# zz9tf/FIA-KDD-19

Hardware: AMD Instinct MI355X
Metric: influence queries/sec (whole node) + % HBM roofline, MF k=16 ML-1M-ex (higher is better)
Workload: dtype f64

## Files before the change

fia-kdd-19_amd/csrc/abi.hip:

```cpp
#include <atomic>
#include <cstdlib>
#include <cstring>
#include <new>

#include "common.h"

namespace fia {

static bool pooled_event(fia_ctx* c, hipEvent_t* e) {
  if (!c->events.pool.empty()) {
    *e = c->events.pool.back();
    c->events.pool.pop_back();
    return true;
  }
  return hipEventCreate(e) == hipSuccess;
}

void phase_begin(fia_ctx* c, int phase, hipStream_t s) {
  if (!(c->profiling >> phase & 1u)) return;
  hipEvent_t a, b;
  if (!pooled_event(c, &a)) return;
  if (!pooled_event(c, &b)) { c->events.pool.push_back(a); return; }
  (void)hipEventRecord(a, s);
  c->events.ev[phase].push_back({a, b});
// ... 178 lines not shown
      if (can_free) b.release(ds);
      else { b.ptr = nullptr; b.bytes = 0; }
    };
    for (int s = 0; s < 2; ++s) {
      for (fia::DevBuf* b : {&c->idx.side[s].ptr, &c->idx.side[s].row, &c->idx.side[s].other, &c->idx.side[s].rating,
                             &c->gram[s], &c->l1[s], &c->idx.order[s], &c->idx.gitems[s], &c->idx.gcomb[s],
                             &c->gpart[s], &c->self[s], &c->gm[s], &c->slot[s], &c->bitems[s], &c->bcomb[s]})
        rel(*b);
    }
    fia::DevBuf* bufs[] = {&c->rec,    &c->coff,   &c->cdesc,    &c->cand_pos,  &c->cand_val, &c->qscan,
                           &c->flag,   &c->nch,    &c->coupled,  &c->idx.pkey,  &c->idx.pcnt, &c->idx.psum,
                           &c->gcnt,   &c->gstart, &c->grank,    &c->gq,        &c->qbase,    &c->gscan,
                           &c->wstart, &c->witems, &c->resid,  &c->qwork,  &c->xb,       &c->syslist,
                           &c->cpllist, &c->lscr, &c->mark, &c->d1tab, &c->slices, &c->wfrag,
                           &c->tkeys, &c->tvals, &c->tagg, &c->tslot, &c->tword, &c->tsort, &c->rowrec, &c->gxq,
                           &c->dwork, &c->dslab, &c->dpairs};
    for (auto* b : bufs) rel(*b);
    if (can_free) (void)hipStreamSynchronize(ds);
    if (c->aux && !capturing) (void)hipStreamDestroy(c->aux);
    if (c->fork_ev) (void)hipEventDestroy(c->fork_ev);
    if (c->l1_ev) (void)hipEventDestroy(c->l1_ev);
    if (c->prep_ev) (void)hipEventDestroy(c->prep_ev);
    for (auto& v : c->events.ev)
      for (auto& pr : v) { (void)hipEventDestroy(pr.first); (void)hipEventDestroy(pr.second); }
    for (auto e : c->events.pool) (void)hipEventDestroy(e);
  }
  if (c->device >= 0 && c->device < kMaxDevices) g_live[c->device].fetch_sub(1);
  delete c;
  return FIA_OK;
}

// ... 628 lines not shown
```

fia-kdd-19_amd/csrc/common.h:

```cpp
#pragma once

#include <hip/hip_runtime.h>
#include <hip/hip_ext.h>
#include <cstdint>
#include <cstdio>
#include <string>
#include <vector>

#include "fia.h"

namespace fia {

constexpr int kWave = 64;
constexpr int kScoreThreads = 256;
constexpr int kScoreRows = 4;
constexpr int kChunk = 64 * kScoreRows;
constexpr int kRunQB = 16;
constexpr int kRunChunk = 128;
constexpr int kNcfRunChunk = 64;
constexpr int kRunUserCost = 3;

struct ChunkDesc {
  int64_t list_base;
  int64_t out_base;
// ... 182 lines not shown
  fia::Params p;
  fia::Index idx;
  fia::DevBuf gram[2];
  fia::DevBuf l1[2];
  fia::DevBuf gpart[2];
  bool prepared = false;
  fia::DevBuf rec;
  fia::DevBuf coff;
  fia::DevBuf cdesc;
  fia::DevBuf cand_pos;
  fia::DevBuf cand_val;
  fia::DevBuf qscan;
  fia::DevBuf flag;
  fia::DevBuf nch;
  fia::DevBuf coupled;
  fia::DevBuf gcnt;
  fia::DevBuf gstart;
  fia::DevBuf grank;
  fia::DevBuf gq;
  fia::DevBuf qbase;
  fia::DevBuf slices;
  fia::DevBuf wstart;
  fia::DevBuf gscan;
  fia::DevBuf witems;
  fia::DevBuf d1tab;
  fia::DevBuf tkeys, tvals, tagg, tslot, tword, tsort;
  fia::DevBuf rowrec, gxq;
  uint64_t rowrec_version = ~0ull;
  fia::DevBuf dwork, dslab, dpairs;
  fia::DevBuf self[2];
// ... 114 lines not shown
  const int2* desc;
  const uint32_t* ids;
  const int32_t* wave;
  int64_t n_waves;
  const float* emb_other[2];
  uint32_t bytes_other[2];
  double* gram[2];
  double* part[2];
  const uint8_t* mark;
  int64_t moff[2];
};
hipError_t launch_gram_mf_stream(int k, const GramStreamArgs& G, hipStream_t s);
hipError_t launch_score_mf_runs(int k, int64_t grid, hipStream_t s, const QueryArgs& A, int64_t Q,
                                const ChunkDesc* cdesc, const int64_t* qbase, const int32_t* slices,
                                const double* rec, int32_t* rel_idx, double* influence, int K, int32_t* cand_pos,
                                double* cand_val, PhaseSpan ps);
hipError_t launch_score_ncf_runs(int k, int64_t grid, hipStream_t s, const QueryArgs& A, int64_t Q,
                                 const ChunkDesc* cdesc, const int64_t* qbase, const int32_t* slices,
                                 const double* rec, int32_t* rel_idx, double* influence, int K, int32_t* cand_pos,
                                 double* cand_val, PhaseSpan ps);
hipError_t launch_score_mf_mfma(int k, bool full, int64_t grid, hipStream_t s, PhaseSpan ps, const QueryArgs& A,
                                int64_t nE, const int64_t* wstart, const int32_t* witems, const int64_t* gstart,
                                const int32_t* gq, const int64_t* qbase, const double* rec, int32_t* rel_idx,
                                double* influence, int K, int32_t* cand_pos, double* cand_val);
hipError_t launch_topk_merge(fia_ctx* c, int64_t Q, const int32_t* qu, const int32_t* qi, int K, int spc,
                             int64_t* topk_pos, int64_t* topk_idx, double* topk_val, hipStream_t s,
                             int64_t max_chunks);

hipError_t score_candidates(fia_ctx* c, int64_t Q, const int32_t* qu, const int32_t* qi, const double* x,
                            const int64_t* cand_offsets, int64_t total_cand, const int32_t* cand_user,
                            const int32_t* cand_item, const float* cand_rating, double* influence, int K,
// ... 74 lines not shown
```

fia-kdd-19_amd/csrc/index.hip:

```cpp
#include <algorithm>
#include <cstdlib>
#include <cstring>
#include <rocprim/device/device_radix_sort.hpp>
#include <rocprim/iterator/counting_iterator.hpp>

#include "common.h"
#include "scan.h"

namespace fia {
namespace {

__global__ void k_check_ids(const int32_t* __restrict__ user, const int32_t* __restrict__ item, int64_t N,
                            int64_t U, int64_t I, int32_t* __restrict__ flag) {
  int64_t j = (int64_t)blockIdx.x * blockDim.x + threadIdx.x;
  int64_t stride = (int64_t)gridDim.x * blockDim.x;
  int bad = 0;
  for (; j < N; j += stride) {
    int32_t u = user[j], i = item[j];
    bad |= (u < 0 || u >= U || i < 0 || i >= I);
  }
  if (__any(bad) && (threadIdx.x & 63) == 0) atomicOr(flag, 1);
}

__global__ void k_gather_side(const int32_t* __restrict__ rows, const int32_t* __restrict__ other_src,
// ... 46 lines not shown
  ub = du = ib = di = 0;
  if (u >= 0 && u < U && i >= 0 && i < I) {
    ub = uptr[u];
    du = uptr[u + 1] - ub;
    ib = iptr[i];
    di = iptr[i + 1] - ib;
  }
}

template <int MODE>
__global__ __launch_bounds__(kScanThreads) void k_query_scan(
    const int32_t* __restrict__ qu, const int32_t* __restrict__ qi, int64_t Q, const int64_t* __restrict__ uptr,
    const int64_t* __restrict__ iptr, int64_t U, int64_t I, int64_t* __restrict__ out,
    unsigned long long* __restrict__ tstate, unsigned int* __restrict__ tctr, int32_t* __restrict__ flag,
    const int64_t* __restrict__ offsets, ChunkDesc* __restrict__ cdesc, int32_t* __restrict__ zero_word,
    int64_t* __restrict__ qbase, int runs, int clen, int lsh, int32_t* __restrict__ slices) {
  query_scan_body<MODE>(qu, qi, Q, uptr, iptr, U, I, out, tstate, tctr, flag, offsets, cdesc, zero_word, qbase, runs,
                        clen, lsh, slices);
}

__global__ void k_group_count(const int32_t* __restrict__ qu, const int32_t* __restrict__ qi, int64_t Q,
                              const int64_t* __restrict__ uptr, const int64_t* __restrict__ iptr, int64_t U, int64_t I,
                              const int64_t* __restrict__ offsets, const int64_t* __restrict__ coff,
                              unsigned long long* __restrict__ gcnt, int32_t* __restrict__ grank,
                              int64_t* __restrict__ qbase) {
  const int64_t q = (int64_t)blockIdx.x * blockDim.x + threadIdx.x;
  if (q >= Q) return;
  int64_t ub, du, ib, di;
  query_sides(qu, qi, q, uptr, iptr, U, I, ub, du, ib, di);
  const int32_t u = qu[q], i = qi[q];
  const bool ok = (u >= 0 && u < U && i >= 0 && i < I) && (du + di > 0);
  grank[2 * q] = ok ? (int32_t)atomicAdd(&gcnt[u], 1ull) : -1;
  grank[2 * q + 1] = ok ? (int32_t)atomicAdd(&gcnt[U + i], 1ull) : -1;
// ... 398 lines not shown
  X.valid = true;
  return hipSuccess;
}

static hipError_t scan_state(fia_ctx* c, int64_t Q, hipStream_t s) {
  const int64_t ntiles = (Q + 1 + kScanTile - 1) / kScanTile;
  const size_t need = sizeof(unsigned long long) * (size_t)(2 * ntiles) + 16;
  if (c->qscan.bytes >= need && c->qscan.ptr) return hipSuccess;
  FIA_HIP_TRY(c->qscan.reserve(need < 4096 ? 4096 : need, s));
  FIA_HIP_TRY(hipMemsetAsync(c->qscan.ptr, 0, c->qscan.bytes, s));
  return hipSuccess;
}

static hipError_t query_scan_args(fia_ctx* c, int64_t Q, const int32_t* qu, const int32_t* qi, int64_t* out,
                                  const int64_t* offsets, ChunkDesc* cdesc, int32_t* zero_word, hipStream_t s,
                                  int64_t* qbase, int runs, int clen, int lsh, int32_t* slices, ScanArgs& S) {
  FIA_HIP_TRY(scan_state(c, Q, s));
  FIA_HIP_TRY(c->flag.reserve(64, s));
  unsigned int* ctr = reinterpret_cast<unsigned int*>(c->qscan.as<char>() + c->qscan.bytes - 16);
  S = ScanArgs{qu, qi, Q, c->idx.side[0].ptr.as<int64_t>(), c->idx.side[1].ptr.as<int64_t>(), c->idx.U, c->idx.I, out,
               c->qscan.as<unsigned long long>(), ctr, c->flag.as<int32_t>(), offsets, cdesc, zero_word, qbase, runs,
               clen, lsh, slices};
  return hipSuccess;
}

template <int MODE>
static hipError_t launch_query_scan(const ScanArgs& S, hipStream_t s, hipEvent_t ev_a, hipEvent_t ev_b) {
  hipExtLaunchKernelGGL(k_query_scan<MODE>, dim3((unsigned)scan_tiles(S.Q)), dim3(kScanThreads), 0, s, ev_a, ev_b, 0,
                        S.qu, S.qi, S.Q, S.uptr, S.iptr, S.U, S.I, S.out, S.tstate, S.tctr, S.flag, S.offsets, S.cdesc,
                        S.zero_word, S.qbase, S.runs, S.clen, S.lsh, S.slices);
  return hipGetLastError();
}

hipError_t count_related(fia_ctx* c, int64_t Q, const int32_t* qu, const int32_t* qi, int64_t* offsets,
                         hipStream_t s) {
  ScanArgs S;
  FIA_HIP_TRY(query_scan_args(c, Q, qu, qi, offsets, nullptr, nullptr, nullptr, s, nullptr, 0, kChunk, 0, nullptr, S));
  return launch_query_scan<0>(S, s, nullptr, nullptr);
}

hipError_t write_related(fia_ctx* c, int64_t Q, const int32_t* qu, const int32_t* qi, const int64_t* offsets,
                         int32_t* rel, hipStream_t s) {
  if (Q == 0) return hipSuccess;
  hipLaunchKernelGGL(k_write_related, dim3((unsigned)Q), dim3(256), 0, s, qu, qi, offsets,
                     c->idx.side[0].ptr.as<int64_t>(), c->idx.side[0].row.as<int32_t>(),
                     c->idx.side[1].ptr.as<int64_t>(), c->idx.side[1].row.as<int32_t>(), c->idx.U, c->idx.I, rel);
  return hipGetLastError();
}


hipError_t chunk_scan_args(fia_ctx* c, int64_t Q, const int32_t* qu, const int32_t* qi, const int64_t* offsets,
                           int64_t max_chunks, bool offsets_only, hipStream_t s, int32_t* zero_word, bool runs,
                           int slice_cost, int run_chunk, ScanArgs& S) {
  FIA_HIP_TRY(c->coff.reserve(sizeof(int64_t) * (size_t)(Q + 1), s));
  const bool rq = runs && !offsets_only;
  if (!offsets_only) FIA_HIP_TRY(c->cdesc.reserve(sizeof(ChunkDesc) * (size_t)(max_chunks + 1), s));
  int lsh = 0;
  while ((1 << lsh) < slice_cost && lsh < 30) ++lsh;
  const int lam = 1 << lsh;
  if (rq) {
    FIA_HIP_TRY(c->qbase.reserve(sizeof(int64_t) * (size_t)(4 * Q + 2), s));
    FIA_HIP_TRY(c->slices.reserve(sizeof(int32_t) * (size_t)((max_chunks + 1) * (kRunQB + 2) / lam + 2), s));
  }
  return query_scan_args(c, Q, qu, qi, c->coff.as<int64_t>(), offsets,
                         offsets_only ? nullptr : c->cdesc.as<ChunkDesc>(), zero_word, s,
                         rq ? c->qbase.as<int64_t>() : nullptr, rq ? kRunQB : 0, rq ? run_chunk : kChunk, lsh,
                         rq ? c->slices.as<int32_t>() : nullptr, S);
}

hipError_t launch_chunk_scan(const ScanArgs& S, hipStream_t s, hipEvent_t ev_a, hipEvent_t ev_b) {
  return launch_query_scan<1>(S, s, ev_a, ev_b);
}

hipError_t build_chunks(fia_ctx* c, int64_t Q, const int32_t* qu, const int32_t* qi, const int64_t* offsets,
                        int64_t max_chunks, bool offsets_only, hipStream_t s, int32_t* zero_word, bool runs,
                        int slice_cost, int run_chunk) {
  ScanArgs S;
  FIA_HIP_TRY(chunk_scan_args(c, Q, qu, qi, offsets, max_chunks, offsets_only, s, zero_word, runs, slice_cost,
                              run_chunk, S));
  return launch_chunk_scan(S, s);
}

// ... 44 lines not shown
```

fia-kdd-19_amd/csrc/models.hip:

```cpp
#include "kern.h"
#include "scan.h"

namespace fia {

QueryArgs make_args(fia_ctx* c, const int32_t* qu, const int32_t* qi) {
  QueryArgs A{};
  fill_list_args(c, A);
  A.qu = qu;
  A.qi = qi;
  A.lgm[0] = c->gm[0].as<double>();
  A.lgm[1] = c->gm[1].as<double>();
  A.lres = c->resid.as<double>();
  A.N = c->idx.N;
  return A;
}

namespace {

template <class M>
constexpr int kModel = M::ncf ? FIA_MODEL_NCF : FIA_MODEL_MF;

constexpr int kRunLambda = 8;

template <class M>
// ... 76 lines not shown
    FIA_HIP_TRY(c->cand_val.reserve(sizeof(double) * (size_t)((max_chunks + 1) * K * spc), s));
  }
  QueryArgs A = make_args(c, qu, qi);
  const int64_t nE = c->idx.U + c->idx.I;
  const int64_t max_items = max_chunks;
  if (c->coupled.bytes < sizeof(int32_t) * (size_t)(Q + 2) || !c->coupled.ptr) {
    FIA_HIP_TRY(c->coupled.reserve(sizeof(int32_t) * (size_t)(Q + 2), s));
    FIA_HIP_TRY(hipMemsetAsync(c->coupled.ptr, 0, c->coupled.bytes, s));
  }
  int32_t* const coupled = c->coupled.as<int32_t>() + 1;
  constexpr bool ext_phases = runs && !M::ncf && use_quad_solve<M>();
  const bool fused = ext_phases && Q > 0 && !x_in;
  if (!ext_phases) phase_begin(c, 4, s);
  constexpr int64_t lam = kRunLambda;
  const int64_t runs_grid = (kRunUserCost * (max_chunks + 1)) / lam + 2;
  ScanArgs S;
  FIA_HIP_TRY(chunk_scan_args(c, Q, qu, qi, offsets, max_chunks, grouped, s, fused ? nullptr : coupled, runs, (int)lam,
                              M::ncf ? kNcfRunChunk : kRunChunk, S));
  if (!fused) {
    const PhaseSpan cspan = ext_phases ? phase_span(c, 4) : PhaseSpan{};
    if (const hipError_t eb = launch_chunk_scan(S, s, cspan.a, cspan.b); eb != hipSuccess) {
      phase_drop(c, 4, cspan);
      return eb;
    }
  }
  if (grouped) FIA_HIP_TRY(build_groups(c, Q, qu, qi, offsets, max_items, qblock, s, use_mfma ? kMfmaCPI : 1));
  if constexpr (pair_layout<M>()) {
    if (Q > 0 && !x_in) {
      FIA_HIP_TRY(join_l1(c, s));
      FIA_HIP_TRY(c->qwork.reserve(sizeof(double) * (size_t)(Q * QPro<M>::stride + 1), s));
      FIA_HIP_TRY(launch_ncf_query_pro(M::K, A, Q, c->qwork.as<double>(), s));
    }
  }
// ... 34 lines not shown
  const PhaseSpan span = phase_span(c, 2);
  if constexpr (grouped) {
    if (use_mfma)
      FIA_HIP_TRY(launch_score_mf_mfma(M::K, rel_idx && influence, grid, s, span, A, nE, c->wstart.as<int64_t>(),
                                       c->witems.as<int32_t>(), c->gstart.as<int64_t>(), c->gq.as<int32_t>(),
                                       c->qbase.as<int64_t>(), c->rec.as<double>(), rel_idx, influence, K,
                                       c->cand_pos.as<int32_t>(), c->cand_val.as<double>()));
    else
      FIA_HIP_TRY(launch_score_grouped(kModel<M>, M::K, grid, s, span, A, nE, c->wstart.as<int64_t>(),
                                       c->witems.as<int32_t>(), c->gstart.as<int64_t>(), c->gq.as<int32_t>(),
                                       c->qbase.as<int64_t>(), c->rec.as<double>(), rel_idx, influence, K,
                                       c->cand_pos.as<int32_t>(), c->cand_val.as<double>()));
  } else if constexpr (!M::ncf) {
    FIA_HIP_TRY(launch_score_mf_runs(M::K, grid, s, A, Q, c->cdesc.as<ChunkDesc>(), c->qbase.as<int64_t>(),
                                     c->slices.as<int32_t>(), c->rec.as<double>(), rel_idx, influence, K,
                                     c->cand_pos.as<int32_t>(), c->cand_val.as<double>(), span));
  } else {
    FIA_HIP_TRY(launch_score_ncf_runs(M::K, grid, s, A, Q, c->cdesc.as<ChunkDesc>(), c->qbase.as<int64_t>(),
                                      c->slices.as<int32_t>(), c->rec.as<double>(), rel_idx, influence, K,
                                      c->cand_pos.as<int32_t>(), c->cand_val.as<double>(), span));
  }
  if (K > 0 && Q > 0) {
    phase_begin(c, 3, s);
    FIA_HIP_TRY(launch_topk_merge(c, Q, qu, qi, K, spc, topk_pos, topk_idx, topk_val, s, max_chunks));
    phase_end(c, 3, s);
  }
  return hipSuccess;
}

}

// ... 100 lines not shown
```

fia-kdd-19_amd/csrc/scan.h:

```cpp
#pragma once

#include "common.h"

namespace fia {

constexpr int kScanThreads = 512, kScanItems = 1, kScanTile = kScanThreads * kScanItems;
constexpr unsigned long long kScanAgg = 1ull << 62, kScanPre = 2ull << 62, kScanVal = (1ull << 62) - 1;

inline int64_t scan_tiles(int64_t Q) { return (Q + 1 + kScanTile - 1) / kScanTile; }

__device__ inline int64_t scan_lookback(unsigned long long* __restrict__ tstate, int64_t tile, int64_t agg) {
  const int lane = threadIdx.x & 63;
  if (lane == 0)
    __hip_atomic_store(&tstate[tile], (tile == 0 ? kScanPre : kScanAgg) | (unsigned long long)agg,
                       __ATOMIC_RELAXED, __HIP_MEMORY_SCOPE_AGENT);
  int64_t excl = 0;
  for (int64_t end = tile - 1; end >= 0;) {
    const int64_t p = end - lane;
    const unsigned long long w =
        p >= 0 ? __hip_atomic_load(&tstate[p], __ATOMIC_RELAXED, __HIP_MEMORY_SCOPE_AGENT) : kScanPre;
    const unsigned long long f = w >> 62;
    const unsigned long long pre = __ballot(f == 2), inv = __ballot(f == 0);
    const int stop = pre ? __builtin_ctzll(pre) : 64;
    const unsigned long long need = stop >= 63 ? ~0ull : ((2ull << stop) - 1);
// ... 5 lines not shown
#pragma unroll
    for (int off = 32; off > 0; off >>= 1) part += __shfl_xor(part, off);
    excl += part;
    if (stop < 64) break;
    end -= 64;
  }
  if (lane == 0 && tile > 0)
    __hip_atomic_store(&tstate[tile], kScanPre | (unsigned long long)(excl + agg), __ATOMIC_RELAXED,
                       __HIP_MEMORY_SCOPE_AGENT);
  return excl;
}

struct ScanFillLds {
  int64_t c0[kScanTile], cost[kScanTile], ub[kScanTile], ib[kScanTile], base[kScanTile];
  int32_t du[kScanTile], di[kScanTile], nq[kScanTile], nd[kScanTile];
  int32_t qi[kScanTile + kRunQB];
  int64_t wave2[kScanThreads / 64], prefix2;
};
template <int MODE>
__device__ __forceinline__ ScanFillLds* scan_fill_lds() {
  if constexpr (MODE == 1) {
    __shared__ ScanFillLds F;
    return &F;
  } else {
    return nullptr;
  }
}

template <int MODE>
__device__ __forceinline__ void query_scan_body(
    const int32_t* __restrict__ qu, const int32_t* __restrict__ qi, int64_t Q, const int64_t* __restrict__ uptr,
    const int64_t* __restrict__ iptr, int64_t U, int64_t I, int64_t* __restrict__ out,
    unsigned long long* __restrict__ tstate, unsigned int* __restrict__ tctr, int32_t* __restrict__ flag,
    const int64_t* __restrict__ offsets, ChunkDesc* __restrict__ cdesc, int32_t* __restrict__ zero_word,
    int64_t* __restrict__ qbase, int runs, int clen, int lsh, int32_t* __restrict__ slices) {
  __shared__ int s_tile;
  __shared__ int64_t s_wave[kScanThreads / 64];
  __shared__ int64_t s_prefix;
  ScanFillLds* const F = scan_fill_lds<MODE>();
  const unsigned ntiles = (unsigned)((Q + 1 + kScanTile - 1) / kScanTile);
  if (threadIdx.x == 0) s_tile = (int)atomicAdd(&tctr[0], 1u);
  __syncthreads();
  const int64_t tile = s_tile;
  const int lane = threadIdx.x & 63, wave = threadIdx.x >> 6;
  const int64_t q0 = tile * kScanTile + (int64_t)threadIdx.x * kScanItems;
  int64_t v[kScanItems];
  int64_t s_ub[kScanItems], s_du[kScanItems], s_ib[kScanItems], s_di[kScanItems], s_base[kScanItems];
  int s_nq[kScanItems];
  int64_t tsum = 0, tsum2 = 0;
  if constexpr (MODE == 1) {
    static_assert(kScanItems == 1, "one query per thread");
    if (runs) {
      const int64_t qa = tile * kScanTile + threadIdx.x;
      F->qi[threadIdx.x] = qa < Q ? qi[qa] : -1;
      if (threadIdx.x < kRunQB) {
        const int64_t qb2 = tile * kScanTile + kScanTile + threadIdx.x;
        F->qi[kScanTile + threadIdx.x] = qb2 < Q ? qi[qb2] : -1;
      }
      __syncthreads();
    }
  }
#pragma unroll
  for (int it = 0; it < kScanItems; ++it) {
    const int64_t q = q0 + it;
    int64_t x = 0;
    s_ub[it] = s_du[it] = s_ib[it] = s_di[it] = s_base[it] = 0;
    s_nq[it] = 0;
    if (q < Q) {
      if (MODE == 1 && cdesc) s_base[it] = offsets[q];
      const int32_t u = qu[q], i = qi[q];
      if (u >= 0 && u < U && i >= 0 && i < I) {
        const int64_t ub = uptr[u], ib = iptr[i];
        const int64_t du = uptr[u + 1] - ub, di = iptr[i + 1] - ib;
        s_ub[it] = ub; s_du[it] = du; s_ib[it] = ib; s_di[it] = di;
        x = MODE == 0 ? du + di : (du + kChunk - 1) / kChunk + (di + kChunk - 1) / kChunk;
        if (MODE == 1 && runs) {
          const int tt = threadIdx.x;
          const bool head = (q % runs) == 0 || (tt > 0 ? F->qi[tt - 1] : qi[q - 1]) != i;
          s_nq[it] = 0;
          if (head) {
            int nq = 1;
            const int lim = runs - (int)(q % runs);
#pragma unroll
            for (int j = 1; j < kRunQB; ++j) {
              const bool same = j < lim && F->qi[tt + j] == i;
              nq += (same && nq == j) ? 1 : 0;
            }
            s_nq[it] = nq;
          }
          const int64_t cu = (du + clen - 1) / clen, ci = (di + clen - 1) / clen;
          x = ((cu + ci) << 31) | (cu + (head ? ci : 0));
          tsum2 += cu * kRunUserCost + (head ? ci * (s_nq[it] + 2) : 0);
        }
      } else if (MODE == 0) {
        atomicOr(flag + 1, 1);
      }
    }
    v[it] = x;
    tsum += x;
  }
  int64_t inc = tsum;
#pragma unroll
  for (int off = 1; off < 64; off <<= 1) {
    const int64_t y = __shfl_up(inc, off);
    if (lane >= off) inc += y;
  }
  int64_t inc2 = tsum2;
// ... 46 lines not shown
      const int64_t du = s_du[it], cr = runs ? run >> 31 : run;
      qbase[4 * q + 0] = s_base[it];
      qbase[4 * q + 1] = s_base[it] + du;
      qbase[4 * q + 2] = cr;
      qbase[4 * q + 3] = cr + (du + clen - 1) / clen;
    }
    if (MODE == 1 && runs) {
      F->c0[threadIdx.x] = run & kLo;
      F->cost[threadIdx.x] = run2;
      F->ub[threadIdx.x] = s_ub[it];
      F->ib[threadIdx.x] = s_ib[it];
      F->base[threadIdx.x] = s_base[it];
      F->du[threadIdx.x] = (int32_t)s_du[it];
      F->di[threadIdx.x] = (int32_t)s_di[it];
      F->nq[threadIdx.x] = s_nq[it];
      F->nd[threadIdx.x] = (q < Q) ? (int32_t)(v[it] & kLo) : 0;
    } else
    if (MODE == 1 && cdesc && q < Q && v[it] > 0) {
      const int64_t ub = s_ub[it], du = s_du[it], ib = s_ib[it], di = s_di[it];
      int64_t c = run;
      const int64_t base = s_base[it];
      for (int64_t st = 0; st < du; st += kChunk, ++c) {
        ChunkDesc d;
        d.list_base = ub + st;
        d.out_base = base + st;
        d.q = (int32_t)q;
        d.pos0 = (int32_t)st;
        d.len = (int32_t)(du - st < kChunk ? du - st : kChunk);
        d.side = 0;
        cdesc[c] = d;
// ... 7 lines not shown
        d.len = (int32_t)(di - st < kChunk ? di - st : kChunk);
        d.side = 1;
        cdesc[c] = d;
      }
    }
    run += v[it];
  }
  if (MODE == 1 && runs && cdesc) {
    __syncthreads();
    const int64_t dstart = F->c0[0], dend = F->c0[kScanTile - 1] + F->nd[kScanTile - 1];
    {
      for (int64_t c = dstart + threadIdx.x; c < dend; c += kScanThreads) {
        const int t = last_at_most(F->c0, 0, kScanTile - 1, c);
        const int64_t j = c - F->c0[t];
        const int32_t du = F->du[t], di = F->di[t], nq = F->nq[t];
        const int64_t cu = (du + clen - 1) / clen;
        const int64_t qq = tile * kScanTile + t;
        ChunkDesc d;
        int64_t p, w;
        if (j < cu) {
          const int64_t st = j * clen;
          d.list_base = F->ub[t] + st;
          d.out_base = F->base[t] + st;
          d.pos0 = (int32_t)st;
          d.len = (int32_t)(du - st < clen ? du - st : clen);
          d.side = 0 | (1 << 8);
          p = F->cost[t] + j * kRunUserCost;
          w = kRunUserCost;
        } else {
          const int64_t st = (j - cu) * clen;
          d.list_base = F->ib[t] + st;
          d.out_base = F->base[t] + du + st;
          d.pos0 = (int32_t)(du + st);
          d.len = (int32_t)(di - st < clen ? di - st : clen);
          d.side = 1 | (nq << 8);
          p = F->cost[t] + cu * kRunUserCost + (j - cu) * (nq + 2);
          w = nq + 2;
        }
        d.q = (int32_t)qq;
        cdesc[c] = d;
        if (slices)
          for (int64_t sl = (p + (1ll << lsh) - 1) >> lsh; (sl << lsh) < p + w; ++sl) slices[sl] = (int32_t)c;
      }
    }
  }
  __syncthreads();
  if (threadIdx.x == 0) {
    asm volatile("s_waitcnt vmcnt(0)" ::: "memory");
    const unsigned done = atomicAdd(&tctr[1], 1u);
    if (done == ntiles - 1) {
      for (unsigned t = 0; t < (MODE == 1 && runs ? 2 * ntiles : ntiles); ++t)
// ... 9 lines not shown
  const int32_t* qi;
  int64_t Q;
  const int64_t* uptr;
  const int64_t* iptr;
  int64_t U, I;
  int64_t* out;
  unsigned long long* tstate;
  unsigned int* tctr;
  int32_t* flag;
  const int64_t* offsets;
  ChunkDesc* cdesc;
  int32_t* zero_word;
  int64_t* qbase;
  int runs, clen, lsh;
  int32_t* slices;
};

template <int MODE>
__device__ __forceinline__ void query_scan_body(const ScanArgs& S) {
  query_scan_body<MODE>(S.qu, S.qi, S.Q, S.uptr, S.iptr, S.U, S.I, S.out, S.tstate, S.tctr, S.flag, S.offsets, S.cdesc,
                        S.zero_word, S.qbase, S.runs, S.clen, S.lsh, S.slices);
}

hipError_t chunk_scan_args(fia_ctx* c, int64_t Q, const int32_t* qu, const int32_t* qi, const int64_t* offsets,
                           int64_t max_chunks, bool offsets_only, hipStream_t s, int32_t* zero_word, bool runs,
                           int slice_cost, int run_chunk, ScanArgs& S);
hipError_t launch_chunk_scan(const ScanArgs& S, hipStream_t s, hipEvent_t ev_a = nullptr, hipEvent_t ev_b = nullptr);

}
```

fia-kdd-19_amd/csrc/score_mf.hip:

```cpp
#include <cstdlib>

#include "kern.h"


namespace fia {

constexpr int kRunsWaves = 3;
namespace {

constexpr int kBufWord3 = 0x00020000;
constexpr int kBufNT = 2;

struct RunArgs {
  const int32_t* other[2];
  const float* rating[2];
  const int32_t* row[2];
  const float* emb_other[2];
  const float* bias_other[2];
};

__device__ __forceinline__ float dpp_maxf(float x, float y) { return x > y ? x : y; }
template <int CTRL>
__device__ __forceinline__ float dpp_max_f32(float m) {
  return dpp_maxf(m, __int_as_float(dpp_i32<CTRL>(__float_as_int(m))));
}
__device__ __forceinline__ void wave_top1_fast(double& a, int& p, double& v) {
  const float k32 = (float)a;
  float m = dpp_max_f32<0x128>(k32);
  m = dpp_max_f32<0x124>(m);
  m = dpp_max_f32<0x122>(m);
  m = dpp_max_f32<0x121>(m);
  m = dpp_maxf(m, __int_as_float((int)other_rows<false>((unsigned)__float_as_int(m))));
  m = dpp_maxf(m, __int_as_float((int)other_rows<true>((unsigned)__float_as_int(m))));
  const unsigned long long who = __ballot(k32 == m);
  if (__builtin_expect(__popcll(who) == 1, 1)) {
    const int l = (int)__builtin_ctzll(who);
    const long long ab = __double_as_longlong(a), vb = __double_as_longlong(v);
    a = __longlong_as_double(((long long)__builtin_amdgcn_readlane((int)(ab >> 32), l) << 32) |
                             (unsigned)__builtin_amdgcn_readlane((int)(ab & 0xffffffffll), l));
    v = __longlong_as_double(((long long)__builtin_amdgcn_readlane((int)(vb >> 32), l) << 32) |
                             (unsigned)__builtin_amdgcn_readlane((int)(vb & 0xffffffffll), l));
    p = __builtin_amdgcn_readlane(p, l);
  } else {
    if (k32 != m) { a = -2.0; p = 0x7fffffff; }
    wave_best(a, p, v);
  }
}

template <class M, int KM>
__global__ __launch_bounds__(64) __attribute__((amdgpu_waves_per_eu(kRunsWaves))) void k_score_mf_runs(
    RunArgs A, int64_t Q, const ChunkDesc* __restrict__ cdesc, const int64_t* __restrict__ qbase,
    const int32_t* __restrict__ slices, const double* __restrict__ rec, int32_t* __restrict__ rel_idx,
    double* __restrict__ influence, int K_top, int32_t* __restrict__ cand_pos, double* __restrict__ cand_val) {
  static_assert(!M::ncf && M::K <= 16 && M::K % 4 == 0, "MF k in {8, 16}");
  constexpr int K = M::K, RT = kRunChunk / 64, NA = K / 4;
  using L = typename M::Rec;
  const int lane = threadIdx.x & 63;
  const int wave = __builtin_amdgcn_readfirstlane(threadIdx.x >> 6);
  const int n_inf = influence ? 8 : 0, n_rel = rel_idx ? 4 : 0;
  const int64_t nsl = qbase[4 * Q + 1];
  const int64_t sl = blockIdx.x;
  if (sl >= nsl) return;
  int64_t ch = slices[sl];
  const int64_t cend = slices[sl + 1];
// ... 11 lines not shown
      const int li = idx < dd.len ? idx : 0;
      o[r] = oth[li];
      y[r] = rat[li];
      rw[r] = rr[li];
    }
  };
  int32_t o[RT], row[RT];
  float y[RT];
  fetch(ch, o, y, row);
  int64_t nx = ch + 1 < cend ? ch + 1 : -1;
  while (true) {
    const ChunkDesc d = cdesc[ch];
    const int sd = d.side & 0xff, nq = d.side >> 8;
    const int32_t q0 = d.q;
    const int len = d.len;
    float4 g4[RT][NA];
    float gb[RT];
    {
      const float* __restrict__ T = A.emb_other[sd];
      const float* __restrict__ bt = A.bias_other[sd];
#pragma unroll
      for (int r = 0; r < RT; ++r) {
        const float4* src = reinterpret_cast<const float4*>(T + (int64_t)o[r] * K);
#pragma unroll
        for (int c = 0; c < NA; ++c) g4[r][c] = src[c];
        gb[r] = bt[o[r]];
      }
    }
    const bool more = nx >= 0;
    int32_t no[RT], nrow[RT];
// ... 33 lines not shown
      const double* __restrict__ Rj = rec + (int64_t)qj * M::R;
      const double* __restrict__ Sj = L::side(Rj, sd);
      const int64_t* __restrict__ qb = qbase + 4 * (int64_t)qj;
#pragma unroll
      for (int c = 0; c < K; ++c) w.x[c] = Sj[L::x + c];
      w.inv_n = Rj[L::inv_n];
      w.cq = Rj[L::c_q];
      w.xsb = Sj[L::x_bias];
      w.dup = Sj[L::dup_other];
      w.ou = qb[0];
      w.oi = qb[1];
      w.slot = qb[2 + sd];
      return w;
    };
    Words wj = words(q0);
    int j = 0;
    do {
      const int32_t qj = q0 + j;
      const double* __restrict__ Rj = rec + (int64_t)qj * M::R;
      double s[RT], s2[RT];
#pragma unroll
      for (int r = 0; r < RT; ++r) s[r] = s2[r] = 0.0;
#pragma unroll
      for (int c = 0; c < K; c += 2) {
        const double xc = wj.x[c], xd = wj.x[c + 1];
#pragma unroll
        for (int r = 0; r < RT; ++r) {
          s[r] = fma(xc, g[r][c], s[r]);
          s2[r] = fma(xd, g[r][c + 1], s2[r]);
        }
      }
#pragma unroll
      for (int r = 0; r < RT; ++r) s[r] += s2[r];
// ... 23 lines not shown
            reinterpret_cast<double*>(reinterpret_cast<uintptr_t>(influence) + (uintptr_t)ob * 8), 0, len * n_inf, kBufWord3);
        const __amdgpu_buffer_rsrc_t rr = __builtin_amdgcn_make_buffer_rsrc(
            reinterpret_cast<int32_t*>(reinterpret_cast<uintptr_t>(rel_idx) + (uintptr_t)ob * 4), 0, len * n_rel, kBufWord3);
#pragma unroll
        for (int r = 0; r < RT; ++r) {
          const int idx = r * 64 + lane;
          const long long ib = __double_as_longlong(infl[r]);
          __builtin_amdgcn_raw_buffer_store_b64(
              (__attribute__((ext_vector_type(2))) unsigned){(unsigned)(ib & 0xffffffffll), (unsigned)(ib >> 32)}, ri,
              idx * 8, 0, kBufNT);
          __builtin_amdgcn_raw_buffer_store_b32((unsigned)row[r], rr, idx * 4, 0, kBufNT);
        }
      }
      const int64_t slot = wj.slot + co / kRunChunk;
      const int32_t pbj = sd ? (int32_t)(oi - ou) : 0;
      wj = words(j + 1 < nq ? qj + 1 : qj);
      if constexpr (KM != 0) {
        if constexpr (KM == 1) {
          double ba = -2.0, bv = 0.0;
          int bp = 0x7fffffff;
#pragma unroll
          for (int r = 0; r < RT; ++r) {
            const int idx = r * 64 + lane;
            const double key = idx < len ? topk_key(infl[r]) : -2.0;
            if (key > ba) { ba = key; bp = idx; bv = infl[r]; }
          }
          wave_top1_fast(ba, bp, bv);
          const bool okk = ba > -1.5;
          const __amdgpu_buffer_rsrc_t rp = __builtin_amdgcn_make_buffer_rsrc(cand_pos + slot, 0, 4, kBufWord3);
          const __amdgpu_buffer_rsrc_t rv = __builtin_amdgcn_make_buffer_rsrc(cand_val + slot, 0, 8, kBufWord3);
          const long long vb = __double_as_longlong(okk ? bv : (double)NAN);
// ... 186 lines not shown
        }
      }
    } while (++j < nq);
    if (!more) break;
    ch = nx;
    nx = ch + 1 < cend ? ch + 1 : -1;
    o = no; y = ny; row = nrow; e = ne; mk = nmk;
  }
}

}

hipError_t launch_score_mf_runs(int k, int64_t grid, hipStream_t s, const QueryArgs& QA, int64_t Q,
                                const ChunkDesc* cdesc, const int64_t* qbase, const int32_t* slices,
                                const double* rec, int32_t* rel_idx, double* influence, int K, int32_t* cand_pos,
                                double* cand_val, PhaseSpan ps) {
  RunArgs A{};
  for (int sd = 0; sd < 2; ++sd) {
    A.other[sd] = QA.other[sd];
    A.rating[sd] = QA.rating[sd];
    A.row[sd] = QA.row[sd];
    A.emb_other[sd] = QA.t[sd == 0 ? 1 : 0];
    A.bias_other[sd] = QA.t[sd == 0 ? 3 : 2];
  }
#define FIA_RUNS_LAUNCH(KK, KM)                                                                                      \
  hipExtLaunchKernelGGL((k_score_mf_runs<MFm<KK>, KM>), dim3((unsigned)grid), dim3(64), 0, s, ps.a, ps.b, 0, A, Q, \
                        cdesc,                                                                                    \
                     qbase, slices, rec, rel_idx, influence, K, cand_pos, cand_val)
  const int km = K <= 0 ? 0 : K == 1 ? 1 : 2;
  if (k == 16) {
    if (km == 0) FIA_RUNS_LAUNCH(16, 0); else if (km == 1) FIA_RUNS_LAUNCH(16, 1); else FIA_RUNS_LAUNCH(16, 2);
  } else if (k == 8) {
    if (km == 0) FIA_RUNS_LAUNCH(8, 0); else if (km == 1) FIA_RUNS_LAUNCH(8, 1); else FIA_RUNS_LAUNCH(8, 2);
  } else {
    return hipErrorInvalidValue;
  }
#undef FIA_RUNS_LAUNCH
  return hipGetLastError();
}

}

namespace fia {

hipError_t launch_score_ncf_runs(int k, int64_t grid, hipStream_t s, const QueryArgs& QA, int64_t Q,
                                 const ChunkDesc* cdesc, const int64_t* qbase, const int32_t* slices,
                                 const double* rec, int32_t* rel_idx, double* influence, int K, int32_t* cand_pos,
                                 double* cand_val, PhaseSpan ps) {
  NcfRunArgs A{};
  for (int sd = 0; sd < 2; ++sd) {
    A.other[sd] = QA.other[sd];
    A.rating[sd] = QA.rating[sd];
// ... 24 lines not shown
```

Measured before the change: 134.4 million.

## Pair queries sharing a user so one user-side chunk pass serves both

A new kernel records, for each user, the first and last query index that references it. The scan then gives the first query's user-side chunks a run of two queries (first and last), drops the last query's user chunks, and adjusts the cost weights. The MF runs kernel walks from the first query to the paired one and resets the pair table in-kernel for the next call. The goal is to avoid streaming the same user's rating list twice. It adds an extra kernel launch, memsets on first use, atomics, and a dirty-state flag across calls, and it only applies to MF with a single live context.

```diff
diff --git a/fia-kdd-19_amd/csrc/abi.hip b/fia-kdd-19_amd/csrc/abi.hip
--- a/fia-kdd-19_amd/csrc/abi.hip
+++ b/fia-kdd-19_amd/csrc/abi.hip
@@ -216,7 +216,7 @@
                            &c->wstart, &c->witems, &c->resid,  &c->qwork,  &c->xb,       &c->syslist,
                            &c->cpllist, &c->lscr, &c->mark, &c->d1tab, &c->slices, &c->wfrag,
                            &c->tkeys, &c->tvals, &c->tagg, &c->tslot, &c->tword, &c->tsort, &c->rowrec, &c->gxq,
-                           &c->dwork, &c->dslab, &c->dpairs};
+                           &c->dwork, &c->dslab, &c->dpairs, &c->upair};
     for (auto* b : bufs) rel(*b);
     if (can_free) (void)hipStreamSynchronize(ds);
     if (c->aux && !capturing) (void)hipStreamDestroy(c->aux);
diff --git a/fia-kdd-19_amd/csrc/common.h b/fia-kdd-19_amd/csrc/common.h
--- a/fia-kdd-19_amd/csrc/common.h
+++ b/fia-kdd-19_amd/csrc/common.h
@@ -220,6 +220,9 @@
   fia::DevBuf flag;
   fia::DevBuf nch;
   fia::DevBuf coupled;
+  fia::DevBuf upair;
+  int64_t upair_cap = 0;
+  bool upair_dirty = false;
   fia::DevBuf gcnt;
   fia::DevBuf gstart;
   fia::DevBuf grank;
@@ -364,7 +367,8 @@
 hipError_t launch_score_mf_runs(int k, int64_t grid, hipStream_t s, const QueryArgs& A, int64_t Q,
                                 const ChunkDesc* cdesc, const int64_t* qbase, const int32_t* slices,
                                 const double* rec, int32_t* rel_idx, double* influence, int K, int32_t* cand_pos,
-                                double* cand_val, PhaseSpan ps);
+                                double* cand_val, PhaseSpan ps, int32_t* ufirst = nullptr,
+                                int32_t* ulast = nullptr);
 hipError_t launch_score_ncf_runs(int k, int64_t grid, hipStream_t s, const QueryArgs& A, int64_t Q,
                                  const ChunkDesc* cdesc, const int64_t* qbase, const int32_t* slices,
                                  const double* rec, int32_t* rel_idx, double* influence, int K, int32_t* cand_pos,
diff --git a/fia-kdd-19_amd/csrc/index.hip b/fia-kdd-19_amd/csrc/index.hip
--- a/fia-kdd-19_amd/csrc/index.hip
+++ b/fia-kdd-19_amd/csrc/index.hip
@@ -84,9 +84,21 @@
     const int64_t* __restrict__ iptr, int64_t U, int64_t I, int64_t* __restrict__ out,
     unsigned long long* __restrict__ tstate, unsigned int* __restrict__ tctr, int32_t* __restrict__ flag,
     const int64_t* __restrict__ offsets, ChunkDesc* __restrict__ cdesc, int32_t* __restrict__ zero_word,
-    int64_t* __restrict__ qbase, int runs, int clen, int lsh, int32_t* __restrict__ slices) {
+    int64_t* __restrict__ qbase, int runs, int clen, int lsh, int32_t* __restrict__ slices,
+    const int32_t* __restrict__ ufirst, const int32_t* __restrict__ ulast) {
   query_scan_body<MODE>(qu, qi, Q, uptr, iptr, U, I, out, tstate, tctr, flag, offsets, cdesc, zero_word, qbase, runs,
-                        clen, lsh, slices);
+                        clen, lsh, slices, ufirst, ulast);
+}
+
+__global__ void k_user_pairs(const int32_t* __restrict__ qu, const int32_t* __restrict__ qi, int64_t Q,
+                             const int64_t* __restrict__ uptr, int64_t U, int64_t I, int32_t* __restrict__ first,
+                             int32_t* __restrict__ last) {
+  const int64_t t = (int64_t)blockIdx.x * blockDim.x + threadIdx.x;
+  if (t >= Q) return;
+  const int32_t u = qu[t], i = qi[t];
+  if (u < 0 || u >= U || i < 0 || i >= I || uptr[u + 1] == uptr[u]) return;
+  atomicMin(&first[u], (int32_t)t);
+  atomicMax(&last[u], (int32_t)t);
 }
 
 __global__ void k_group_count(const int32_t* __restrict__ qu, const int32_t* __restrict__ qi, int64_t Q,
@@ -515,13 +527,14 @@
 
 static hipError_t query_scan_args(fia_ctx* c, int64_t Q, const int32_t* qu, const int32_t* qi, int64_t* out,
                                   const int64_t* offsets, ChunkDesc* cdesc, int32_t* zero_word, hipStream_t s,
-                                  int64_t* qbase, int runs, int clen, int lsh, int32_t* slices, ScanArgs& S) {
+                                  int64_t* qbase, int runs, int clen, int lsh, int32_t* slices, ScanArgs& S,
+                                  const int32_t* ufirst = nullptr, const int32_t* ulast = nullptr) {
   FIA_HIP_TRY(scan_state(c, Q, s));
   FIA_HIP_TRY(c->flag.reserve(64, s));
   unsigned int* ctr = reinterpret_cast<unsigned int*>(c->qscan.as<char>() + c->qscan.bytes - 16);
   S = ScanArgs{qu, qi, Q, c->idx.side[0].ptr.as<int64_t>(), c->idx.side[1].ptr.as<int64_t>(), c->idx.U, c->idx.I, out,
                c->qscan.as<unsigned long long>(), ctr, c->flag.as<int32_t>(), offsets, cdesc, zero_word, qbase, runs,
-               clen, lsh, slices};
+               clen, lsh, slices, ufirst, ulast};
   return hipSuccess;
 }
 
@@ -529,7 +542,7 @@
 static hipError_t launch_query_scan(const ScanArgs& S, hipStream_t s, hipEvent_t ev_a, hipEvent_t ev_b) {
   hipExtLaunchKernelGGL(k_query_scan<MODE>, dim3((unsigned)scan_tiles(S.Q)), dim3(kScanThreads), 0, s, ev_a, ev_b, 0,
                         S.qu, S.qi, S.Q, S.uptr, S.iptr, S.U, S.I, S.out, S.tstate, S.tctr, S.flag, S.offsets, S.cdesc,
-                        S.zero_word, S.qbase, S.runs, S.clen, S.lsh, S.slices);
+                        S.zero_word, S.qbase, S.runs, S.clen, S.lsh, S.slices, S.ufirst, S.ulast);
   return hipGetLastError();
 }
 
@@ -550,9 +563,23 @@
 }
 
 
+static hipError_t reserve_user_pairs(fia_ctx* c, hipStream_t s) {
+  const int64_t U = c->idx.U > 0 ? c->idx.U : 1;
+  if (c->upair.ptr && c->upair_cap >= U && !c->upair_dirty) return hipSuccess;
+  if (!c->upair.ptr || c->upair_cap < U) {
+    FIA_HIP_TRY(c->upair.reserve(sizeof(int32_t) * (size_t)(2 * U), s));
+    c->upair_cap = (int64_t)(c->upair.bytes / (2 * sizeof(int32_t)));
+  }
+  FIA_HIP_TRY(hipMemsetD32Async(reinterpret_cast<hipDeviceptr_t>(c->upair.ptr), kPairNoFirst, (size_t)c->upair_cap, s));
+  FIA_HIP_TRY(hipMemsetD32Async(reinterpret_cast<hipDeviceptr_t>(c->upair.as<int32_t>() + c->upair_cap), kPairNoLast,
+                                (size_t)c->upair_cap, s));
+  c->upair_dirty = false;
+  return hipSuccess;
+}
+
 hipError_t chunk_scan_args(fia_ctx* c, int64_t Q, const int32_t* qu, const int32_t* qi, const int64_t* offsets,
                            int64_t max_chunks, bool offsets_only, hipStream_t s, int32_t* zero_word, bool runs,
-                           int slice_cost, int run_chunk, ScanArgs& S) {
+                           int slice_cost, int run_chunk, ScanArgs& S, bool pairs) {
   FIA_HIP_TRY(c->coff.reserve(sizeof(int64_t) * (size_t)(Q + 1), s));
   const bool rq = runs && !offsets_only;
   if (!offsets_only) FIA_HIP_TRY(c->cdesc.reserve(sizeof(ChunkDesc) * (size_t)(max_chunks + 1), s));
@@ -563,10 +590,21 @@
     FIA_HIP_TRY(c->qbase.reserve(sizeof(int64_t) * (size_t)(4 * Q + 2), s));
     FIA_HIP_TRY(c->slices.reserve(sizeof(int32_t) * (size_t)((max_chunks + 1) * (kRunQB + 2) / lam + 2), s));
   }
+  const bool up = rq && pairs;
+  if (up) FIA_HIP_TRY(reserve_user_pairs(c, s));
   return query_scan_args(c, Q, qu, qi, c->coff.as<int64_t>(), offsets,
                          offsets_only ? nullptr : c->cdesc.as<ChunkDesc>(), zero_word, s,
                          rq ? c->qbase.as<int64_t>() : nullptr, rq ? kRunQB : 0, rq ? run_chunk : kChunk, lsh,
-                         rq ? c->slices.as<int32_t>() : nullptr, S);
+                         rq ? c->slices.as<int32_t>() : nullptr, S, up ? c->upair.as<int32_t>() : nullptr,
+                         up ? c->upair.as<int32_t>() + c->upair_cap : nullptr);
+}
+
+hipError_t launch_user_pairs(fia_ctx* c, const ScanArgs& S, hipStream_t s) {
+  if (!S.ufirst || S.Q <= 0) return hipSuccess;
+  c->upair_dirty = true;
+  hipLaunchKernelGGL(k_user_pairs, dim3((unsigned)((S.Q + 255) / 256)), dim3(256), 0, s, S.qu, S.qi, S.Q, S.uptr, S.U,
+                     S.I, const_cast<int32_t*>(S.ufirst), const_cast<int32_t*>(S.ulast));
+  return hipGetLastError();
 }
 
 hipError_t launch_chunk_scan(const ScanArgs& S, hipStream_t s, hipEvent_t ev_a, hipEvent_t ev_b) {
diff --git a/fia-kdd-19_amd/csrc/models.hip b/fia-kdd-19_amd/csrc/models.hip
--- a/fia-kdd-19_amd/csrc/models.hip
+++ b/fia-kdd-19_amd/csrc/models.hip
@@ -114,9 +114,11 @@
   if (!ext_phases) phase_begin(c, 4, s);
   constexpr int64_t lam = kRunLambda;
   const int64_t runs_grid = (kRunUserCost * (max_chunks + 1)) / lam + 2;
+  const bool pairs = runs && !M::ncf && Q > 0 && !x_in && live_contexts(c->device) <= 1;
   ScanArgs S;
   FIA_HIP_TRY(chunk_scan_args(c, Q, qu, qi, offsets, max_chunks, grouped, s, fused ? nullptr : coupled, runs, (int)lam,
-                              M::ncf ? kNcfRunChunk : kRunChunk, S));
+                              M::ncf ? kNcfRunChunk : kRunChunk, S, pairs));
+  if (pairs) FIA_HIP_TRY(launch_user_pairs(c, S, s));
   if (!fused) {
     const PhaseSpan cspan = ext_phases ? phase_span(c, 4) : PhaseSpan{};
     if (const hipError_t eb = launch_chunk_scan(S, s, cspan.a, cspan.b); eb != hipSuccess) {
@@ -181,7 +183,9 @@
   } else if constexpr (!M::ncf) {
     FIA_HIP_TRY(launch_score_mf_runs(M::K, grid, s, A, Q, c->cdesc.as<ChunkDesc>(), c->qbase.as<int64_t>(),
                                      c->slices.as<int32_t>(), c->rec.as<double>(), rel_idx, influence, K,
-                                     c->cand_pos.as<int32_t>(), c->cand_val.as<double>(), span));
+                                     c->cand_pos.as<int32_t>(), c->cand_val.as<double>(), span,
+                                     const_cast<int32_t*>(S.ufirst), const_cast<int32_t*>(S.ulast)));
+    if (S.ufirst) user_pairs_done(c);
   } else {
     FIA_HIP_TRY(launch_score_ncf_runs(M::K, grid, s, A, Q, c->cdesc.as<ChunkDesc>(), c->qbase.as<int64_t>(),
                                       c->slices.as<int32_t>(), c->rec.as<double>(), rel_idx, influence, K,
diff --git a/fia-kdd-19_amd/csrc/scan.h b/fia-kdd-19_amd/csrc/scan.h
--- a/fia-kdd-19_amd/csrc/scan.h
+++ b/fia-kdd-19_amd/csrc/scan.h
@@ -43,6 +43,7 @@
 struct ScanFillLds {
   int64_t c0[kScanTile], cost[kScanTile], ub[kScanTile], ib[kScanTile], base[kScanTile];
   int32_t du[kScanTile], di[kScanTile], nq[kScanTile], nd[kScanTile];
+  int32_t up[kScanTile];
   int32_t qi[kScanTile + kRunQB];
   int64_t wave2[kScanThreads / 64], prefix2;
 };
@@ -56,13 +57,17 @@
   }
 }
 
+constexpr int32_t kPairNoFirst = 0x7fffffff, kPairNoLast = -1;
+constexpr int32_t kUserSolo = -1, kUserNone = -2;
+
 template <int MODE>
 __device__ __forceinline__ void query_scan_body(
     const int32_t* __restrict__ qu, const int32_t* __restrict__ qi, int64_t Q, const int64_t* __restrict__ uptr,
     const int64_t* __restrict__ iptr, int64_t U, int64_t I, int64_t* __restrict__ out,
     unsigned long long* __restrict__ tstate, unsigned int* __restrict__ tctr, int32_t* __restrict__ flag,
     const int64_t* __restrict__ offsets, ChunkDesc* __restrict__ cdesc, int32_t* __restrict__ zero_word,
-    int64_t* __restrict__ qbase, int runs, int clen, int lsh, int32_t* __restrict__ slices) {
+    int64_t* __restrict__ qbase, int runs, int clen, int lsh, int32_t* __restrict__ slices,
+    const int32_t* __restrict__ ufirst, const int32_t* __restrict__ ulast) {
   __shared__ int s_tile;
   __shared__ int64_t s_wave[kScanThreads / 64];
   __shared__ int64_t s_prefix;
@@ -76,15 +81,16 @@
   int64_t v[kScanItems];
   int64_t s_ub[kScanItems], s_du[kScanItems], s_ib[kScanItems], s_di[kScanItems], s_base[kScanItems];
   int s_nq[kScanItems];
+  int32_t s_up[kScanItems];
   int64_t tsum = 0, tsum2 = 0;
   if constexpr (MODE == 1) {
     static_assert(kScanItems == 1, "one query per thread");
     if (runs) {
       const int64_t qa = tile * kScanTile + threadIdx.x;
-      F->qi[threadIdx.x] = qa < Q ? qi[qa] : -1;
+      F->qi[threadIdx.x] = qa < Q && qu[qa] >= 0 && qu[qa] < U ? qi[qa] : -1;
       if (threadIdx.x < kRunQB) {
         const int64_t qb2 = tile * kScanTile + kScanTile + threadIdx.x;
-        F->qi[kScanTile + threadIdx.x] = qb2 < Q ? qi[qb2] : -1;
+        F->qi[kScanTile + threadIdx.x] = qb2 < Q && qu[qb2] >= 0 && qu[qb2] < U ? qi[qb2] : -1;
       }
       __syncthreads();
     }
@@ -95,6 +101,7 @@
     int64_t x = 0;
     s_ub[it] = s_du[it] = s_ib[it] = s_di[it] = s_base[it] = 0;
     s_nq[it] = 0;
+    s_up[it] = kUserSolo;
     if (q < Q) {
       if (MODE == 1 && cdesc) s_base[it] = offsets[q];
       const int32_t u = qu[q], i = qi[q];
@@ -118,8 +125,19 @@
             s_nq[it] = nq;
           }
           const int64_t cu = (du + clen - 1) / clen, ci = (di + clen - 1) / clen;
-          x = ((cu + ci) << 31) | (cu + (head ? ci : 0));
-          tsum2 += cu * kRunUserCost + (head ? ci * (s_nq[it] + 2) : 0);
+          int nu = 1;
+          if (ufirst && du > 0) {
+            const int32_t f = ufirst[u], l = ulast[u];
+            if (f == (int32_t)q) {
+              if (l != f) { s_up[it] = l; nu = 2; }
+            } else if (l == (int32_t)q) {
+              s_up[it] = kUserNone;
+            }
+          }
+          static_assert(kRunUserCost == 2 + 1, "a user-side run of one");
+          const int64_t cuw = s_up[it] == kUserNone ? 0 : cu;
+          x = ((cu + ci) << 31) | (cuw + (head ? ci : 0));
+          tsum2 += cuw * (2 + nu) + (head ? ci * (s_nq[it] + 2) : 0);
         }
       } else if (MODE == 0) {
         atomicOr(flag + 1, 1);
@@ -196,6 +214,7 @@
       F->du[threadIdx.x] = (int32_t)s_du[it];
       F->di[threadIdx.x] = (int32_t)s_di[it];
       F->nq[threadIdx.x] = s_nq[it];
+      F->up[threadIdx.x] = s_up[it];
       F->nd[threadIdx.x] = (q < Q) ? (int32_t)(v[it] & kLo) : 0;
     } else
     if (MODE == 1 && cdesc && q < Q && v[it] > 0) {
@@ -233,7 +252,9 @@
         const int t = last_at_most(F->c0, 0, kScanTile - 1, c);
         const int64_t j = c - F->c0[t];
         const int32_t du = F->du[t], di = F->di[t], nq = F->nq[t];
-        const int64_t cu = (du + clen - 1) / clen;
+        const int32_t up = F->up[t];
+        const int nu = up >= 0 ? 2 : 1;
+        const int64_t cu = up == kUserNone ? 0 : (du + clen - 1) / clen;
         const int64_t qq = tile * kScanTile + t;
         ChunkDesc d;
         int64_t p, w;
@@ -241,11 +262,11 @@
           const int64_t st = j * clen;
           d.list_base = F->ub[t] + st;
           d.out_base = F->base[t] + st;
-          d.pos0 = (int32_t)st;
+          d.pos0 = nu == 2 ? up : (int32_t)st;
           d.len = (int32_t)(du - st < clen ? du - st : clen);
-          d.side = 0 | (1 << 8);
-          p = F->cost[t] + j * kRunUserCost;
-          w = kRunUserCost;
+          d.side = 0 | (nu << 8);
+          p = F->cost[t] + j * (2 + nu);
+          w = 2 + nu;
         } else {
           const int64_t st = (j - cu) * clen;
           d.list_base = F->ib[t] + st;
@@ -253,7 +274,7 @@
           d.pos0 = (int32_t)(du + st);
           d.len = (int32_t)(di - st < clen ? di - st : clen);
           d.side = 1 | (nq << 8);
-          p = F->cost[t] + cu * kRunUserCost + (j - cu) * (nq + 2);
+          p = F->cost[t] + cu * (2 + nu) + (j - cu) * (nq + 2);
           w = nq + 2;
         }
         d.q = (int32_t)qq;
@@ -293,17 +314,21 @@
   int64_t* qbase;
   int runs, clen, lsh;
   int32_t* slices;
+  const int32_t* ufirst;
+  const int32_t* ulast;
 };
 
 template <int MODE>
 __device__ __forceinline__ void query_scan_body(const ScanArgs& S) {
   query_scan_body<MODE>(S.qu, S.qi, S.Q, S.uptr, S.iptr, S.U, S.I, S.out, S.tstate, S.tctr, S.flag, S.offsets, S.cdesc,
-                        S.zero_word, S.qbase, S.runs, S.clen, S.lsh, S.slices);
+                        S.zero_word, S.qbase, S.runs, S.clen, S.lsh, S.slices, S.ufirst, S.ulast);
 }
 
 hipError_t chunk_scan_args(fia_ctx* c, int64_t Q, const int32_t* qu, const int32_t* qi, const int64_t* offsets,
                            int64_t max_chunks, bool offsets_only, hipStream_t s, int32_t* zero_word, bool runs,
-                           int slice_cost, int run_chunk, ScanArgs& S);
+                           int slice_cost, int run_chunk, ScanArgs& S, bool pairs = false);
+hipError_t launch_user_pairs(fia_ctx* c, const ScanArgs& S, hipStream_t s);
+inline void user_pairs_done(fia_ctx* c) { c->upair_dirty = false; }
 hipError_t launch_chunk_scan(const ScanArgs& S, hipStream_t s, hipEvent_t ev_a = nullptr, hipEvent_t ev_b = nullptr);
 
 }
diff --git a/fia-kdd-19_amd/csrc/score_mf.hip b/fia-kdd-19_amd/csrc/score_mf.hip
--- a/fia-kdd-19_amd/csrc/score_mf.hip
+++ b/fia-kdd-19_amd/csrc/score_mf.hip
@@ -17,6 +17,9 @@
   const int32_t* row[2];
   const float* emb_other[2];
   const float* bias_other[2];
+  const int32_t* qu;
+  int32_t* ufirst;
+  int32_t* ulast;
 };
 
 __device__ __forceinline__ float dpp_maxf(float x, float y) { return x > y ? x : y; }
@@ -47,7 +50,7 @@
   }
 }
 
-template <class M, int KM>
+template <class M, int KM, bool PAIR>
 __global__ __launch_bounds__(64) __attribute__((amdgpu_waves_per_eu(kRunsWaves))) void k_score_mf_runs(
     RunArgs A, int64_t Q, const ChunkDesc* __restrict__ cdesc, const int64_t* __restrict__ qbase,
     const int32_t* __restrict__ slices, const double* __restrict__ rec, int32_t* __restrict__ rel_idx,
@@ -89,6 +92,16 @@
     const int sd = d.side & 0xff, nq = d.side >> 8;
     const int32_t q0 = d.q;
     const int len = d.len;
+    if constexpr (PAIR) {
+      const int32_t uq = A.qu[q0];
+      const int rs = (sd == 0 && d.out_base == qbase[4 * (int64_t)q0]) ? 4 : 0;
+      const __amdgpu_buffer_rsrc_t rf = __builtin_amdgcn_make_buffer_rsrc(
+          reinterpret_cast<int32_t*>(reinterpret_cast<uintptr_t>(A.ufirst) + (uintptr_t)uq * 4), 0, rs, kBufWord3);
+      const __amdgpu_buffer_rsrc_t rl = __builtin_amdgcn_make_buffer_rsrc(
+          reinterpret_cast<int32_t*>(reinterpret_cast<uintptr_t>(A.ulast) + (uintptr_t)uq * 4), 0, rs, kBufWord3);
+      __builtin_amdgcn_raw_buffer_store_b32(0x7fffffffu, rf, lane * 4, 0, 0);
+      __builtin_amdgcn_raw_buffer_store_b32(0xffffffffu, rl, lane * 4, 0, 0);
+    }
     float4 g4[RT][NA];
     float gb[RT];
     {
@@ -152,9 +165,9 @@
       return w;
     };
     Words wj = words(q0);
+    int32_t qj = q0;
     int j = 0;
     do {
-      const int32_t qj = q0 + j;
       const double* __restrict__ Rj = rec + (int64_t)qj * M::R;
       double s[RT], s2[RT];
 #pragma unroll
@@ -208,7 +221,8 @@
       }
       const int64_t slot = wj.slot + co / kRunChunk;
       const int32_t pbj = sd ? (int32_t)(oi - ou) : 0;
-      wj = words(j + 1 < nq ? qj + 1 : qj);
+      qj = j + 1 < nq ? ((!PAIR || sd) ? qj + 1 : d.pos0) : qj;
+      wj = words(qj);
       if constexpr (KM != 0) {
         if constexpr (KM == 1) {
           double ba = -2.0, bv = 0.0;
@@ -425,8 +439,11 @@
 hipError_t launch_score_mf_runs(int k, int64_t grid, hipStream_t s, const QueryArgs& QA, int64_t Q,
                                 const ChunkDesc* cdesc, const int64_t* qbase, const int32_t* slices,
                                 const double* rec, int32_t* rel_idx, double* influence, int K, int32_t* cand_pos,
-                                double* cand_val, PhaseSpan ps) {
+                                double* cand_val, PhaseSpan ps, int32_t* ufirst, int32_t* ulast) {
   RunArgs A{};
+  A.qu = QA.qu;
+  A.ufirst = ufirst;
+  A.ulast = ulast;
   for (int sd = 0; sd < 2; ++sd) {
     A.other[sd] = QA.other[sd];
     A.rating[sd] = QA.rating[sd];
@@ -434,10 +451,13 @@
     A.emb_other[sd] = QA.t[sd == 0 ? 1 : 0];
     A.bias_other[sd] = QA.t[sd == 0 ? 3 : 2];
   }
-#define FIA_RUNS_LAUNCH(KK, KM)                                                                                      \
-  hipExtLaunchKernelGGL((k_score_mf_runs<MFm<KK>, KM>), dim3((unsigned)grid), dim3(64), 0, s, ps.a, ps.b, 0, A, Q, \
-                        cdesc,                                                                                    \
-                     qbase, slices, rec, rel_idx, influence, K, cand_pos, cand_val)
+#define FIA_RUNS_LAUNCH1(KK, KM, PAIR)                                                                              \
+  hipExtLaunchKernelGGL((k_score_mf_runs<MFm<KK>, KM, PAIR>), dim3((unsigned)grid), dim3(64), 0, s, ps.a, ps.b, 0, \
+                        A, Q, cdesc, qbase, slices, rec, rel_idx, influence, K, cand_pos, cand_val)
+#define FIA_RUNS_LAUNCH(KK, KM)                                            \
+  do {                                                                     \
+    if (ufirst) FIA_RUNS_LAUNCH1(KK, KM, true); else FIA_RUNS_LAUNCH1(KK, KM, false); \
+  } while (0)
   const int km = K <= 0 ? 0 : K == 1 ? 1 : 2;
   if (k == 16) {
     if (km == 0) FIA_RUNS_LAUNCH(16, 0); else if (km == 1) FIA_RUNS_LAUNCH(16, 1); else FIA_RUNS_LAUNCH(16, 2);
@@ -447,6 +467,7 @@
     return hipErrorInvalidValue;
   }
 #undef FIA_RUNS_LAUNCH
+#undef FIA_RUNS_LAUNCH1
   return hipGetLastError();
 }
 
```

Result: no change. 133.2 million (-0.9%).
